# balbasty/torch-interpol

Hardware: AMD Instinct MI355X
Metric: Mvox/s grid_pull & grid_push, 256^3 fp32 cubic/dct2 (higher is better)
Workload: dtype f32

## Files before the change

torch-interpol_amd/csrc/push_owner.hip:

```cpp
#include "sorted_util.hpp"

namespace ip {
namespace owner {

using namespace sorted;

constexpr int BR = 16;
constexpr int OFF = 160;
constexpr int BOX = BR + 3;
constexpr int PZ = BOX;
constexpr int PLANE = BOX * PZ;
constexpr int BOXSLOTS = BOX * PLANE;
constexpr int NCELL = BR * BR * BR;
constexpr int CAPD = 128;
constexpr int CAPX = 512;
constexpr int NT = 512;
constexpr int NS = TS * TS * TS;
constexpr int NT1 = 512, VPT1 = NS / NT1;
constexpr int LB = 6, NBIN = LB * LB * LB;
constexpr int HDR_SHELL = 34;
constexpr int KMIX = 13;
template <int K> constexpr int KSV = K == KMIX ? 3 : K;
template <int K> __device__ __forceinline__ int kd(const KParams &p, int d) { return K == KMIX ? p.order[d] : K; }
#ifdef IP_OWNER_MIX_TU
// ... 870 lines not shown
#pragma unroll
        for (int d = 0; d < 3; ++d) wsum3 *= kd<K>(p, d) == 3 ? 1.6666667f : (kd<K>(p, d) == 2 ? 1.75f : 2.f);
        const bool dense = n >= 60000 || (float)(sm.dmax * foldmul) * wsum3 > 2147483648.f * 0.99f / magic_units_p<K>(p);
#else
        const float wsum = K == 3 ? 1.6666667f : (K == 2 ? 1.75f : 2.f);
        const bool dense = n >= 60000 || (float)(sm.dmax * foldmul) * (wsum * wsum * wsum) > magic_cbmax<K>();
#endif
        const bool one_batch = npieces <= NPIECE;
        for (int c = 0; c < nch; c += 2) {
            const bool two = c + 1 < nch;
            float *vc0 = vol + b * p.vol_sb + c * p.vol_sc;
            float *vc1 = two ? vc0 + p.vol_sc : vc0;
            const float *va = c == 0 ? nullptr : vals + (int64_t)(c - 1) * nrec;
            const float *vb = two ? vals + (int64_t)c * nrec : nullptr;
            if (c > 0) {
                float am0 = 0.f, am1 = 0.f;
                for (int e = tid; e < NCELL / 2; e += NT) sm.cells[e] = 0u;
                __syncthreads();
                for (int pb0 = 0; pb0 < npieces; pb0 += NPIECE) {
                    if (!one_batch) { __syncthreads(); build_pieces(pb0); }
                    for (int k = 0; k < VPT; ++k) {
                        const uint2 pc = sm.piece[wave + k * (NT / 64)];
                        if (lane >= (int)pc.y) continue;
                        const unsigned ri = pc.x + (unsigned)lane;
                        const int cell = (int)(meta[ri] & 4095u);
                        atomicAdd(&sm.cells[cell >> 1], 1u << (16 * (cell & 1)));
                        const float a0 = __builtin_fabsf(va[ri]), a1 = two ? __builtin_fabsf(vb[ri]) : 0.f;
                        am0 = (a0 > am0 || a0 != a0) ? a0 : am0;
                        am1 = (a1 > am1 || a1 != a1) ? a1 : am1;
                    }
                }
                const int w0 = wave_max(__float_as_int(am0)), w1 = wave_max(__float_as_int(am1));
                if (lane == 0) { if (w0) atomicMax(&sm.cmax[0], w0); if (w1) atomicMax(&sm.cmax[1], w1); }
                __syncthreads();
            }
            const int mb0 = sm.cmax[0], mb1 = sm.cmax[1];
            const bool fin = (mb0 & 0x7f800000) != 0x7f800000 && (mb1 & 0x7f800000) != 0x7f800000;
            const bool wide = dense && fin;
            const bool fixedpt = fin && !(p.dbg & 8);
            int ex0 = ((mb0 >> 23) & 0xff) - 127, ex1 = ((mb1 >> 23) & 0xff) - 127;
            ex0 = ex0 < -90 ? -90 : ex0; ex1 = ex1 < -90 ? -90 : ex1;
            const float a0 = fmaxf(__int_as_float(mb0), 1e-27f), a1 = fmaxf(__int_as_float(mb1), 1e-27f);
            const f2 scale = { mb0 ? IP_MU / a0 : 0.f, mb1 ? IP_MU / a1 : 0.f };
            const float inv0 = a0 * (1.f / IP_MU), inv1 = a1 * (1.f / IP_MU);
            const f2 scalew = { mb0 ? __int_as_float((127 + 30 - ex0) << 23) : 0.f, mb1 ? __int_as_float((127 + 30 - ex1) << 23) : 0.f };
            const float invw0 = __int_as_float((127 - 30 + ex0) << 23), invw1 = __int_as_float((127 - 30 + ex1) << 23);
            const unsigned boxaddr = (unsigned)(size_t)(__attribute__((address_space(3))) void *)(sm.box);
            for (int sub = 0; sub < (wide && two ? 2 : 1); ++sub) {
            for (int pb0 = 0; pb0 < npieces; pb0 += NPIECE) {
                const int tid = opaque((int)threadIdx.x);
                const int wave = tid >> 6, lane = tid & 63;
                if (pb0 > 0 || c > 0 || sub > 0) {
                    __syncthreads();
                    if (tid < NCLS) sm.qcnt[tid] = 0;
                    if (!one_batch) build_pieces(pb0); else __syncthreads();
#pragma unroll
                    for (int k = 0; k < VPT; ++k) {
                        const uint2 pc = sm.piece[wave + k * (NT / 64)];
                        qr[k] = -1;
                        if (lane < (int)pc.y) {
                            const unsigned mk = meta[pc.x + (unsigned)lane];
                            const int x0 = (mk >> 8) & 15, y0 = (mk >> 4) & 15, z0 = mk & 15;
                            const int q = (x0 * PLANE + y0 * PZ + z0) & (NCLS - 1);
                            qr[k] = q | (atomicAdd(&sm.qcnt[q], 1) << 4);
                        }
                    }
                    __syncthreads();
                } else if (!one_batch) {
                    __syncthreads();
                    build_pieces(0);
                }
                if (tid < 32) {
                    const bool cls = tid < NCLS;
                    const int cq = cls ? sm.qcnt[tid] : 0;
                    int tot, nsur, nhol;
                    half_excl_scan(cq, tot);
                    const int cap = (((tot + NCLS - 1) / NCLS) + NHW - 1) / NHW * NHW;
                    const int sur = cls && cq > cap ? cq - cap : 0, hol = cls && cq < cap ? cap - cq : 0;
                    const int so = half_excl_scan(sur, nsur), ho = half_excl_scan(hol, nhol);
                    if (cls) { sm.qsur[tid] = so; sm.qhol[tid] = ho; }
                    if (tid == 31) { sm.qsur[NCLS] = nsur; sm.qhol[NCLS] = nhol; sm.qcap = cap; }
                    const int fill = nsur - ho < 0 ? 0 : (nsur - ho > hol ? hol : nsur - ho);
                    if (cls) sm.qeff[tid] = (cq < cap ? cq : cap) + fill;
                }
                __syncthreads();
                const int qcap = sm.qcap;
#pragma unroll
                for (int k = 0; k < VPT; ++k) {
                    if (qr[k] < 0) continue;
                    const int qq = qr[k] & (NCLS - 1), r = qr[k] >> 4;
                    int slot = qq * qcap + r;
                    if (r >= qcap) {
                        const int o = sm.qsur[qq] + r - qcap;
                        int c2 = 0;
#pragma unroll
                        for (int st = NCLS / 2; st > 0; st >>= 1) if (sm.qhol[c2 + st] <= o) c2 += st;
                        slot = c2 * qcap + sm.qcnt[c2] + (o - sm.qhol[c2]);
                    }
                    sm.queue[slot] = (unsigned short)(((wave + k * (NT / 64)) << 6) | lane);
                }
                __syncthreads();
                const int q = tid & (NCLS - 1), hw = tid >> 4;
                const int ebeg = q * qcap + hw, eend = q * qcap + sm.qeff[q];
                const int nit = qcap / NHW;
                auto fetch = [&](int e, float4 &rc, float &s0, float &s1) {
                    const unsigned qe = sm.queue[e];
                    const unsigned ri = sm.piece[qe >> 6].x + (qe & 63u);
                    rc = rec[ri]; s0 = va ? va[ri] : rc.w; s1 = vb ? vb[ri] : 0.f;
                };
                float4 rc = make_float4(0.f, 0.f, 0.f, 0.f); float s0 = 0.f, s1 = 0.f;
                if (ebeg < eend) fetch(ebeg, rc, s0, s1);
#pragma unroll 1
                for (int it = 0; it < nit; ++it) {
                    const int e = ebeg + it * NHW;
                    const float4 cur = rc; const float cs0 = s0, cs1 = s1;
                    if (e + NHW < eend) fetch(e + NHW, rc, s0, s1);
                    if (e >= eend) continue;
                    int x0, y0, z0; float tx, ty, tz;
                    IP_RECORD_CELL(cur, b0, x0, y0, z0, tx, ty, tz);
                    if (fixedpt) {
#ifdef IP_ABLATE
                        if (p.dbg & 2) continue;
#endif
                        unsigned addr = boxaddr + 8u * (unsigned)(x0 * PLANE + y0 * PZ + z0);
                        f2 w[4];
#ifdef IP_OWNER_MIX_TU
                        if constexpr (K == KMIX) mixed_weights_yz(p.order[1], p.order[2], f2{ ty, tz }, w);
                        else
#endif
                        weights_yz<K>(f2{ ty, tz }, w);
                        if (wide) {
                            const f2 ss = sub ? f2{ cs1 * scalew.y, 0.f } : f2{ cs0 * scalew.x, 0.f };
                            scatter_plane<K, 0, true>(addr, ss, IP_WX(0), w, p.dbg);
                            scatter_plane<K, 1, true>(addr, ss, IP_WX(1), w, p.dbg);
                            if (IP_KS >= 2) scatter_plane<K, 2, true>(addr, ss, IP_WX(2), w, p.dbg);
                            if (IP_KS == 3) scatter_plane<K, 3, true>(addr, ss, IP_WX(3), w, p.dbg);
                        } else {
                            const f2 ss = f2{ cs0, cs1 } * scale;
                            scatter_plane<K, 0, false>(addr, ss, IP_WX(0), w, p.dbg);
                            scatter_plane<K, 1, false>(addr, ss, IP_WX(1), w, p.dbg);
                            if (IP_KS >= 2) scatter_plane<K, 2, false>(addr, ss, IP_WX(2), w, p.dbg);
                            if (IP_KS == 3) scatter_plane<K, 3, false>(addr, ss, IP_WX(3), w, p.dbg);
                        }
                    } else {
                        tiled::scatter_one_thread(L, vc0, cs0, b0[0] + x0, b0[1] + y0, b0[2] + z0, tx, ty, tz);
                        if (two) tiled::scatter_one_thread(L, vc1, cs1, b0[0] + x0, b0[1] + y0, b0[2] + z0, tx, ty, tz);
                    }
                }
            }
            asm volatile("s_waitcnt lgkmcnt(0)" ::: "memory");
            __syncthreads();
            prof_mark(11);
            const bool magic = fixedpt && !wide;
            if (magic) stencil_counts<K>(sm, tid);
            prof_mark(13);
            if (edge && fixedpt) {
#pragma unroll
                for (int d = 0; d < 3; ++d) {
                    const int nlo = b0[d] < 0 ? -b0[d] : 0, nhi = b0[d] + BOX > L.n[d] ? b0[d] + BOX - L.n[d] : 0;
                    if (nlo + nhi == 0) continue;
                    for (int i = tid; i < (nlo + nhi) * (BOX * BOX); i += NT) {
                        const int o = i / (BOX * BOX), rest = i - o * (BOX * BOX), r1 = rest / BOX, r2 = rest - r1 * BOX;
                        const int rd = o < nlo ? o : BOX - nhi + (o - nlo);
                        const int idx = b0[d] + rd;
                        int j;
                        if (L.bound[d] == B_REPLICATE) j = idx < 0 ? 0 : L.n[d] - 1;
                        else if (L.bound[d] == B_DCT1) j = idx < 0 ? -idx : 2 * L.n[d] - 2 - idx;
                        else j = idx < 0 ? -1 - idx : 2 * L.n[d] - 1 - idx;
                        const int rt = j - b0[d];
                        const int es = d == 0 ? rd * PLANE + r1 * PZ + r2 : d == 1 ? r1 * PLANE + rd * PZ + r2 : r1 * PLANE + r2 * PZ + rd;
                        const int et = d == 0 ? rt * PLANE + r1 * PZ + r2 : d == 1 ? r1 * PLANE + rt * PZ + r2 : r1 * PLANE + r2 * PZ + rt;
                        const unsigned long long v = sm.box[es];
                        if (v) { sm.box[es] = 0ull; atomicAdd(&sm.box[et], v); }
                        if (magic) {
                            const int ns = d == 0 ? (rd * BOX + r1) * NZ + r2 : d == 1 ? (r1 * BOX + rd) * NZ + r2 : (r1 * BOX + r2) * NZ + rd;
                            const int nt = d == 0 ? (rt * BOX + r1) * NZ + r2 : d == 1 ? (r1 * BOX + rt) * NZ + r2 : (r1 * BOX + r2) * NZ + rt;
                            unsigned short *nn = reinterpret_cast<unsigned short *>(sm.nreg);
                            const unsigned c2 = nn[ns];
                            if (c2) { nn[ns] = 0; atomicAdd(&sm.nreg[nt >> 1], c2 << (16 * (nt & 1))); }
                        }
                    }
                    __syncthreads();
                }
            }
            if (fixedpt && !atomic && !wide && !(p.dbg & 1)) {
                constexpr int UF2 = 7;
#pragma unroll 1
                for (int e0 = tid; e0 < BOXSLOTS; e0 += UF2 * NT) {
                    int off[UF2]; float t0[UF2], t1[UF2];
                    unsigned nz = 0, nst[UF2];
#pragma unroll
                    for (int u = 0; u < UF2; ++u) {
                        const int e = e0 + u * NT;
                        off[u] = 0;
                        if (e < BOXSLOTS) {
                            const int xr = e / PLANE, rem = e - xr * PLANE, yr = rem / PZ, zr = rem - yr * PZ;
                            off[u] = (b0[0] + xr) * L.ss[0] + (b0[1] + yr) * L.ss[1] + (b0[2] + zr) * L.ss[2];
                            nst[u] = stencils_at(sm, xr, yr, zr);
                            if (nst[u] != 0u) nz |= 1u << u;
                        }
                    }
#pragma unroll
                    for (int u = 0; u < UF2; ++u) {
                        t0[u] = ((nz >> u) & 1) ? vc0[off[u]] : 0.f;
                        t1[u] = (((nz >> u) & 1) && two) ? vc1[off[u]] : 0.f;
                    }
#pragma unroll
                    for (int u = 0; u < UF2; ++u) {
                        if (!((nz >> u) & 1)) continue;
                        const int e = e0 + u * NT;
                        const unsigned long long a = sm.box[e];
                        sm.box[e] = 0ull;
                        int lo_, hi_;
                        magic_decode(a, nst[u], lo_, hi_);
                        vc0[off[u]] = t0[u] + (float)lo_ * inv0;
                        if (two) vc1[off[u]] = t1[u] + (float)hi_ * inv1;
                    }
                }
            } else if (fixedpt && !(p.dbg & 1)) {
                constexpr int UF = 4;
                const int fl0 = atomic ? sm.rlo[0] : 0, fl1 = atomic ? sm.rlo[1] : 0, fl2 = atomic ? sm.rlo[2] : 0;
                const int fe1 = atomic ? sm.rhi[1] + IP_KS - fl1 + 1 : BOX, fe2 = atomic ? sm.rhi[2] + IP_KS - fl2 + 1 : BOX;
                const int nflush = atomic ? (sm.rhi[0] + IP_KS - fl0 + 1) * fe1 * fe2 : BOXSLOTS;
                const float r2 = 1.f / (float)fe2, r1 = 1.f / (float)fe1;
                for (int e0 = tid; e0 < nflush; e0 += UF * NT) {
                    long long a[UF]; int off[UF]; float sg[UF]; unsigned nst[UF];
#pragma unroll
                    for (int u = 0; u < UF; ++u) {
                        int e = e0 + u * NT;
                        a[u] = 0; off[u] = 0; sg[u] = 1.f; nst[u] = 0u;
                        if (e < nflush) {
                            int xr, yr, zr;
                            if (atomic) {
                                const int t = (int)(((float)e + 0.5f) * r2);
                                zr = e - t * fe2 + fl2;
                                xr = (int)(((float)t + 0.5f) * r1);
                                yr = t - xr * fe1 + fl1; xr += fl0;
                                e = xr * PLANE + yr * PZ + zr;
                            } else {
                                xr = e / PLANE; const int rem = e - xr * PLANE; yr = rem / PZ; zr = rem - yr * PZ;
                            }
                            a[u] = (long long)sm.box[e];
                            sm.box[e] = 0ull;
                            if (!wide) nst[u] = stencils_at(sm, xr, yr, zr);
                            if (atomic) {
                                off[u] = sm.taboff[0][xr] + sm.taboff[1][yr] + sm.taboff[2][zr];
                                sg[u] = sm.tabsgn[0][xr] * sm.tabsgn[1][yr] * sm.tabsgn[2][zr];
                            } else {
                                off[u] = (b0[0] + xr) * L.ss[0] + (b0[1] + yr) * L.ss[1] + (b0[2] + zr) * L.ss[2];
                            }
                        }
                    }
                    if (wide) {
                        float *vcs = sub ? vc1 : vc0;
                        const float invs = sub ? invw1 : invw0;
#pragma unroll
                        for (int u = 0; u < UF; ++u) {
                            if (a[u] == 0) continue;
                            const float val = (float)((double)a[u] * (double)(invs * sg[u]));
                            if (atomic) __hip_atomic_fetch_add(vcs + off[u], val, __ATOMIC_RELAXED, __HIP_MEMORY_SCOPE_AGENT);
                            else vcs[off[u]] += val;
                        }
                    } else if (atomic) {
#pragma unroll
                        for (int u = 0; u < UF; ++u) {
                            if (nst[u] == 0u) continue;
                            int lo_, hi_;
                            magic_decode((unsigned long long)a[u], nst[u], lo_, hi_);
                            if (lo_ != 0) __hip_atomic_fetch_add(vc0 + off[u], (float)lo_ * (inv0 * sg[u]), __ATOMIC_RELAXED, __HIP_MEMORY_SCOPE_AGENT);
                            if (hi_ != 0 && two) __hip_atomic_fetch_add(vc1 + off[u], (float)hi_ * (inv1 * sg[u]), __ATOMIC_RELAXED, __HIP_MEMORY_SCOPE_AGENT);
                        }
                    } else {
                        float t0[UF], t1[UF];
#pragma unroll
                        for (int u = 0; u < UF; ++u) {
                            t0[u] = nst[u] != 0u ? vc0[off[u]] : 0.f;
                            t1[u] = (nst[u] != 0u && two) ? vc1[off[u]] : 0.f;
                        }
#pragma unroll
                        for (int u = 0; u < UF; ++u) {
                            if (nst[u] == 0u) continue;
                            int lo_, hi_;
                            magic_decode((unsigned long long)a[u], nst[u], lo_, hi_);
                            vc0[off[u]] = t0[u] + (float)lo_ * inv0;
                            if (two) vc1[off[u]] = t1[u] + (float)hi_ * inv1;
                        }
                    }
                }
            }
            __syncthreads();
            }
            prof_mark(12);
            if (tid == 0) { sm.cmax[0] = 0; sm.cmax[1] = 0; }
        }
    }
    }
}

static __global__ void own_zero(int *__restrict__ p, int n)
{
    const int i = blockIdx.x * 1024 + threadIdx.x;
    if (i < n) p[i] = 0;
}


constexpr int GPZ = 20;
constexpr int GPLANE = BOX * GPZ;
struct GatSmem {
    int   taboff[3][BOX + 1];
    float tabsgn[3][BOX + 1];
    unsigned start[CAPD];
    int   pref[CAPD + 2];
    int   brick, pad;
    float2 box[BOX * GPLANE];
};
#define IP_RD(o, off) "ds_read_b64 %" #o ", %16 offset:" #off "\n\t"
__device__ __forceinline__ void gather_reads(unsigned addr, f2 (&v)[16])
{
    static_assert(GPZ * 8 == 160, "the immediate offsets are (row * GPZ + k) * 8");
    asm volatile(IP_RD(0, 0) IP_RD(1, 8) IP_RD(2, 16) IP_RD(3, 24)
                 IP_RD(4, 160) IP_RD(5, 168) IP_RD(6, 176) IP_RD(7, 184)
                 IP_RD(8, 320) IP_RD(9, 328) IP_RD(10, 336) IP_RD(11, 344)
                 IP_RD(12, 480) IP_RD(13, 488) IP_RD(14, 496) IP_RD(15, 504)
                 "s_waitcnt lgkmcnt(0)"
                 : "=&v"(v[0]), "=&v"(v[1]), "=&v"(v[2]), "=&v"(v[3]), "=&v"(v[4]), "=&v"(v[5]), "=&v"(v[6]), "=&v"(v[7]),
                   "=&v"(v[8]), "=&v"(v[9]), "=&v"(v[10]), "=&v"(v[11]), "=&v"(v[12]), "=&v"(v[13]), "=&v"(v[14]), "=&v"(v[15])
                 : "v"(addr) : "memory");
}
#undef IP_RD

template <int K, int GRAD = 0>
__global__ __launch_bounds__(NT, 4) void own_gather(KParams p, BrickGrid bg, const int *__restrict__ ndesc, const uint2 *__restrict__ desc,
                                                    const float4 *__restrict__ rec, const int *__restrict__ list, int *__restrict__ draw,
                                                    const float *__restrict__ img, float *__restrict__ out, const int *__restrict__ gate,
                                                    const float *__restrict__ gout)
{
    if (gate && *gate != 1) return;
    extern __shared__ __attribute__((aligned(16))) unsigned char smem_raw[];
    GatSmem &sm = *reinterpret_cast<GatSmem *>(smem_raw);
    const int nlist = list[0];
    for (;;) {
// ... 238 lines not shown
        if (!((valid >> v) & 1)) continue;
#pragma unroll
        for (int d = 0; d < 3; ++d) {
            const int i = fl[v][d] == fl[v][d] ? __float2int_rz(fl[v][d]) : 0;
            mn[d] = i < mn[d] ? i : mn[d]; mx[d] = i > mx[d] ? i : mx[d];
            if ((corner >> v) & 1) { atomicMin(&clo[d], i); atomicMax(&chi[d], i); }
        }
    }
#pragma unroll
    for (int d = 0; d < 3; ++d) {
        const int a = wave_min(mn[d]), e = wave_max(mx[d]);
        if ((tid & 63) == 0) { atomicMin(&lo[d], a); atomicMax(&hi[d], e); }
    }
    __syncthreads();
    const int cap[3] = { 33, 33, 32 };
    int l[3], h[3], boxvol = 1, cornervol = 1;
#pragma unroll
    for (int d = 0; d < 3; ++d) {
        int a = lo[d], sz = hi[d] + K - a + 1;
        if (sz > cap[d]) { a += (sz - cap[d]) / 2; sz = cap[d]; }
        l[d] = a; h[d] = a + sz - K - 1;
        boxvol *= sz > 0 ? sz : 0;
        const int cs = chi[d] + K - clo[d] + 1;
        cornervol *= cs > 0 ? (cs < cap[d] ? cs : cap[d]) : 0;
    }
    int slow = 0, nv = 0;
#pragma unroll
    for (int v = 0; v < VPT1; ++v) {
        if (!((valid >> v) & 1)) continue;
        ++nv;
        bool in = true;
#pragma unroll
        for (int d = 0; d < 3; ++d) {
            const int i = fl[v][d] == fl[v][d] ? __float2int_rz(fl[v][d]) : 0x7fffffff;
            in = in && i >= l[d] && i <= h[d];
        }
        if (!in) ++slow;
    }
    slow = wave_sum(slow); far = wave_sum(far); nv = wave_sum(nv);
    if ((tid & 63) == 0) { atomicAdd(&cnt[0], slow); atomicAdd(&cnt[1], far); atomicAdd(&cnt[2], nv); }
    __syncthreads();
    if (tid == 0) {
        atomicAdd(&hdr->nslow, cnt[0]); atomicAdd(&hdr->nfar, cnt[1]); atomicAdd(&hdr->nvalid, cnt[2]);
        if (cnt[2] == NS) { atomicAdd(&hdr->nbox, boxvol); atomicAdd(&hdr->nfull, 1); atomicAdd(&hdr->ncorner, cornervol); }
        __threadfence();
        if (atomicAdd(&hdr->done, 1) == (int)gridDim.x - 1) {
            const int ns = atomicAdd(&hdr->nslow, 0), nf = atomicAdd(&hdr->nfar, 0), nn = atomicAdd(&hdr->nvalid, 0);
            const int nb = atomicAdd(&hdr->nbox, 0), nt = atomicAdd(&hdr->nfull, 0), nc = atomicAdd(&hdr->ncorner, 0);
            const bool rough = nch > 1 && (int64_t)nb > (int64_t)BOXVOL * nt && (int64_t)nb * 10 > (int64_t)nc * 16;
            const bool dense = (int64_t)nc <= (int64_t)DENSEVOL * nt;
            if (nch == -2) hdr->gate = ((int64_t)ns * 1000 > (int64_t)nn * PULLOUT && (int64_t)nf * 64 <= nn) ? 1 : 0;
            else if (nch < 0) hdr->gate = (((int64_t)ns * 250 > nn || dense) && (int64_t)nf * 64 <= nn) ? 1 : 0;
            else hdr->gate = (((int64_t)ns * 250 > nn || rough) && (int64_t)nf * 64 <= nn) ? 1 : 0;
        }
    }
}

struct Workspace {
    int *flags;
    ProbeHdr *hdr; int *ndesc; int *bmax; uint2 *desc; float4 *rec; float *vals; unsigned short *meta;
    int64_t nrec; int nbricks;
};
static int64_t align256(int64_t x) { return (x + 255) & ~(int64_t)255; }

static int64_t layout(const KParams &k, int B, int ntiles, int nch, void *base, Workspace *w, int64_t nflags = 0, bool shared = false)
{
    const BrickGrid bg = brick_grid(k);
    const int64_t nbricks = (int64_t)bg.per_item * (shared ? 1 : B);
    const int64_t nrec = (int64_t)ntiles * NS * B;
    int64_t o = 0;
    unsigned char *p = (unsigned char *)base;
    const int64_t o_hdr = o; o += 256;
    const int64_t o_nd = o; o += nbricks * 4;
    const int64_t o_bm = o; o += nbricks * 8;
    const int64_t o_fl = o; o += nflags * 4; o = align256(o);
    const int64_t o_desc = o; o += align256(nbricks * (shared ? CAPX : CAPD) * 8);
    const int64_t o_rec = o; o += align256(nrec * 16);
    const int64_t o_val = o; o += align256(nrec * 4 * (nch > 1 ? nch - 1 : 0));
    const int64_t o_meta = o; o += align256(nrec * 2);
    if (w) {
        w->hdr = (ProbeHdr *)(p + o_hdr); w->ndesc = (int *)(p + o_nd); w->desc = (uint2 *)(p + o_desc);
        w->rec = (float4 *)(p + o_rec); w->vals = (float *)(p + o_val); w->meta = (unsigned short *)(p + o_meta);
        w->bmax = (int *)(p + o_bm); w->flags = (int *)(p + o_fl);
        w->nrec = nrec; w->nbricks = (int)nbricks;
    }
    return o;
}

static int tile_count(const interpol_problem *p)
{
    int64_t n = 1;
    for (int d = 0; d < 3; ++d) n *= (p->grid_shape[d] + TS - 1) / TS;
    return n > 0x7fffffff ? 0 : (int)n;
}

int mix_launch_bin(int dtype, int idx, const KParams &k, const BrickGrid &bg, const Workspace &w, const void *val, const void *grid, void *vol,
                   const int *gate, const void *aux, const int *all, int gx, int gy, int gz, int ntiles, int B, hipStream_t st);
int mix_launch_acc(const KParams &k, const BrickGrid &bg, const Workspace &w, void *vol, int nch, int color, int Bw, const int *gate,
                   unsigned nblocks, hipStream_t st);
int mix_launch_gather(int grad, const KParams &k, const BrickGrid &bg, const Workspace &w, const void *vol, void *val, const int *gate,
                      const void *gout, unsigned nblocks, hipStream_t st);

#ifdef IP_OWNER_MIX_TU
int mix_launch_bin(int dtype, int idx, const KParams &k, const BrickGrid &bg, const Workspace &w, const void *val, const void *grid, void *vol,
                   const int *gate, const void *aux, const int *all, int gx, int gy, int gz, int ntiles, int B, hipStream_t st)
{
    const int nty = (gy + TS - 1) / TS, ntz = (gz + TS - 1) / TS;
    const dim3 tgrid((unsigned)(ntiles * B));
#define IP_MIX_BIN(T, IDX)                                                                                              \
    {                                                                                                                   \
        const int attr = big_lds<own_bin<T, KMIX, 0, IDX>>(sizeof(BinSmem));                                            \
        if (attr) return attr;                                                                                          \
        hipLaunchKernelGGL((own_bin<T, KMIX, 0, IDX>), tgrid, dim3(NT1), sizeof(BinSmem), st, k, bg, (const T *)val, (const float *)grid, \
                           (float *)vol, w.ndesc, w.desc, w.rec, w.vals, w.meta, w.bmax, w.nrec, gx, gy, gz, nty, ntz, ntiles, gate, (const T *)aux, all); \
    }
    if (idx == 0) { if (dtype == INTERPOL_F32) IP_MIX_BIN(float, 0) else if (dtype == INTERPOL_BF16) IP_MIX_BIN(bf16_t, 0) else if (dtype == INTERPOL_F16) IP_MIX_BIN(f16_t, 0) else return INTERPOL_E_DTYPE; }
    else if (idx == 1) IP_MIX_BIN(float, 1) else if (idx == 2) IP_MIX_BIN(float, 2) else IP_MIX_BIN(float, 3)
#undef IP_MIX_BIN
    const hipError_t e = hipGetLastError();
    return e == hipSuccess ? 0 : (int)e;
}
int mix_launch_acc(const KParams &k, const BrickGrid &bg, const Workspace &w, void *vol, int nch, int color, int Bw, const int *gate,
                   unsigned nblocks, hipStream_t st)
{
    const int attr = big_lds<own_accumulate<KMIX>>(sizeof(AccSmem));
    if (attr) return attr;
    hipLaunchKernelGGL((own_accumulate<KMIX>), dim3(nblocks), dim3(NT), sizeof(AccSmem), st, k, bg, (const int *)w.ndesc,
                       (const uint2 *)w.desc, (const float4 *)w.rec, (const float *)w.vals, (const unsigned short *)w.meta,
                       (const int *)w.bmax, w.nrec, (float *)vol, nch, color, Bw, gate, (int *)w.hdr + 16 + color);
    const hipError_t e = hipGetLastError();
    return e == hipSuccess ? 0 : (int)e;
}
int mix_launch_gather(int grad, const KParams &k, const BrickGrid &bg, const Workspace &w, const void *vol, void *val, const int *gate,
                      const void *gout, unsigned nblocks, hipStream_t st)
{
#define IP_MIX_GAT(GR)                                                                                                  \
    {                                                                                                                   \
        const int attr = big_lds<own_gather<KMIX, GR>>(sizeof(GatSmem));                                                \
        if (attr) return attr;                                                                                          \
        hipLaunchKernelGGL((own_gather<KMIX, GR>), dim3(nblocks), dim3(NT), sizeof(GatSmem), st, k, bg, (const int *)w.ndesc, (const uint2 *)w.desc, \
                           (const float4 *)w.rec, (const int *)w.bmax, (int *)w.hdr + 40, (const float *)vol, (float *)val, gate, (const float *)gout); \
    }
    if (grad == 1) IP_MIX_GAT(1) else if (grad == 2) IP_MIX_GAT(2) else IP_MIX_GAT(0)
#undef IP_MIX_GAT
    const hipError_t e = hipGetLastError();
    return e == hipSuccess ? 0 : (int)e;
}
#endif

}

#ifndef IP_OWNER_MIX_TU

static bool shared_target(const interpol_problem *p) { return p->vol_stride[0] == 0 && p->batch > 1; }
static bool mixed_orders(const KParams &k) { return k.order[0] != k.order[1] || k.order[0] != k.order[2]; }
static bool owner_eligible(const interpol_problem *p, const KParams &k, bool scatter = false)
{
    const bool shared = scatter && shared_target(p);
    if (p->dim != 3 || p->batch > 4096) return false;
    if (!(p->flags & (INTERPOL_FLAG_BINNED_SCATTER | INTERPOL_FLAG_AUTO_SCATTER))) return false;
    if (k.order[0] != k.order[1] || k.order[0] != k.order[2]) {
        for (int d = 0; d < 3; ++d) if (k.order[d] < 1 || k.order[d] > 3) return false;
        if (k.sep != 0) return false;
    } else if (k.order[0] < (scatter ? 1 : 2) || k.order[0] > 3) return false;
    int64_t n = 1, nv = 1, nb = shared ? 1 : p->batch;
    for (int d = 0; d < 3; ++d) {
        n *= p->grid_shape[d]; nv *= p->vol_shape[d];
        nb *= owner::NLO + owner::NHI + (p->vol_shape[d] + 15 + owner::BR - 1) / owner::BR;
        if (p->grid_shape[d] > 0x7fffffff / 4) return false;
    }
    const int64_t nt = owner::tile_count(p);
    if (n < 4096 || nt == 0 || nt * owner::NS * p->batch > 0x7fffffffll || nb > 0x7fffffffll / (shared ? owner::CAPX : owner::CAPD)) return false;
    if ((uint64_t)n * 12ull > 0xffffffffull) return false;
    return (shared ? 8 * n * p->batch : 4 * n) >= nv;
}

int linear_pull_probe(const interpol_problem *p, const KParams &k, const void *grid, void *workspace, hipStream_t st, const int **gate_out, int thr16);
constexpr int NEAREST_THR16 = 24;
static bool nearest_scatter(const KParams &k) { return k.dim == 3 && k.mode == MODE_ISO0 && k.order[0] == 0 && k.order[1] == 0 && k.order[2] == 0; }
static KParams nearest_as_trilinear(const KParams &k)
{
    KParams q = k;
    if (nearest_scatter(k)) { q.order[0] = 1; q.order[1] = 1; q.order[2] = 1; }
    return q;
}

int64_t owner_workspace_bytes(const interpol_problem *p, const KParams &k_in, bool count_only)
{
    const KParams k = nearest_as_trilinear(k_in);
    if (!owner_eligible(p, k, true)) return 0;
    const int nch = count_only ? 1 : k.C + (k.cc ? 1 : 0);
    return owner::layout(k, (int)p->batch, owner::tile_count(p), nch, nullptr, nullptr, 0, shared_target(p));
}

namespace owner {
template <typename T, int IDX = 0>
static int launch_bin(const interpol_problem *p, const KParams &k, const BrickGrid &bg, const Workspace &w, const void *val, const void *grid,
                      void *vol, const int *gate, hipStream_t st, const void *aux = nullptr, const int *all = nullptr)
{
    const int gx = (int)p->grid_shape[0], gy = (int)p->grid_shape[1], gz = (int)p->grid_shape[2];
    const int nty = (gy + TS - 1) / TS, ntz = (gz + TS - 1) / TS;
    const int ntiles = tile_count(p);
    const dim3 tgrid((unsigned)(ntiles * (int)p->batch));
    if (k.order[0] != k.order[1] || k.order[0] != k.order[2])
        return mix_launch_bin(std::is_same<T, float>::value ? INTERPOL_F32 : (std::is_same<T, bf16_t>::value ? INTERPOL_BF16 : INTERPOL_F16), IDX, k, bg, w,
                              val, grid, vol, gate, aux, all, gx, gy, gz, ntiles, (int)p->batch, st);
#define IP_OWN_BIN(KK, GM)                                                                                              \
    {                                                                                                                   \
        const int attr = big_lds<own_bin<T, KK, GM, IDX>>(sizeof(BinSmem));                                               \
        if (attr) return attr;                                                                                          \
        hipLaunchKernelGGL((own_bin<T, KK, GM, IDX>), tgrid, dim3(NT1), sizeof(BinSmem), st, k, bg, (const T *)val, (const float *)grid, \
                           (float *)vol, w.ndesc, w.desc, w.rec, w.vals, w.meta, w.bmax, w.nrec, gx, gy, gz, nty, ntz, ntiles, gate, (const T *)aux, all); \
    }
#define IP_OWN_BY_GM(KK)                                                                                                \
    { if (k.sep == 0) IP_OWN_BIN(KK, 0) else if (k.sep == 1) IP_OWN_BIN(KK, 1) else if (k.sep == 2) IP_OWN_BIN(KK, 2) else IP_OWN_BIN(KK, 3) }
    if (k.order[0] == 3) IP_OWN_BY_GM(3) else if (k.order[0] == 2) IP_OWN_BY_GM(2) else IP_OWN_BY_GM(1)
#undef IP_OWN_BY_GM
#undef IP_OWN_BIN
    return 0;
}
}

int try_owner_push(const interpol_problem *p, const KParams &k_in, const void *val, const void *grid, void *vol,
                   void *workspace, int64_t workspace_bytes, hipStream_t st, const int **gate_out)
{
    using namespace owner;
    const bool nearest = nearest_scatter(k_in);
    const KParams k = nearest_as_trilinear(k_in);
    if (!workspace || !owner_eligible(p, k, true)) return 0;
    const bool count_only = val == nullptr;
    const int nch = count_only ? 1 : k.C + (k.cc ? 1 : 0);
    Workspace w;
    if (((uintptr_t)workspace & 255u) != 0) return 0;
    const bool shared = shared_target(p);
    if (layout(k, (int)p->batch, tile_count(p), nch, workspace, &w, 0, shared) > workspace_bytes) return 0;
    BrickGrid bg = brick_grid(k);
    if (shared) { bg.item = 0; bg.capd = CAPX; }
    const bool gated = !(p->flags & INTERPOL_FLAG_BINNED_SCATTER);
    if (nearest && gated && k.sep != 0 && k.sep != 2) return 0;
    hipLaunchKernelGGL(own_zero, dim3((unsigned)((64 + 3ll * w.nbricks + 1023) / 1024)), dim3(1024), 0, st, (int *)w.hdr, 64 + 3 * w.nbricks);
    hipError_t e = hipGetLastError();
    if (e != hipSuccess) return (int)e;
    const int *gate = nullptr;
    const int B = (int)p->batch;
    if (gated && nearest) {
        const int rp = linear_pull_probe(p, k, grid, w.hdr, st, &gate, NEAREST_THR16);
        if (rp) return rp;
    } else if (gated) {
        const int gx = (int)p->grid_shape[0], gy = (int)p->grid_shape[1], gz = (int)p->grid_shape[2];
        const int nty = (gy + TS - 1) / TS, ntz = (gz + TS - 1) / TS, ntiles = tile_count(p);
        const long long total = (long long)ntiles * B;
        const dim3 pgrid((unsigned)(total < NPROBE ? total : NPROBE));
#define IP_OWN_PROBE(KK, GM) hipLaunchKernelGGL((own_probe<KK, GM>), pgrid, dim3(NT1), 0, st, k, bg, (const float *)grid, w.hdr, gx, gy, gz, nty, ntz, ntiles, B, nch);
#define IP_OWN_PROBE_GM(KK) { if (k.sep == 0) IP_OWN_PROBE(KK, 0) else if (k.sep == 1) IP_OWN_PROBE(KK, 1) else if (k.sep == 2) IP_OWN_PROBE(KK, 2) else IP_OWN_PROBE(KK, 3) }
        if (k.order[0] == 3 || mixed_orders(k)) IP_OWN_PROBE_GM(3) else if (k.order[0] == 2) IP_OWN_PROBE_GM(2) else IP_OWN_PROBE_GM(1)
#undef IP_OWN_PROBE_GM
#undef IP_OWN_PROBE
        gate = &w.hdr->gate;
    }
    int rc;
    switch (count_only ? INTERPOL_F32 : p->dtype) {
    case INTERPOL_F32: rc = launch_bin<float>(p, k, bg, w, val, grid, vol, gate, st); break;
    case INTERPOL_BF16: rc = launch_bin<bf16_t>(p, k, bg, w, val, grid, vol, gate, st); break;
    case INTERPOL_F16: rc = launch_bin<f16_t>(p, k, bg, w, val, grid, vol, gate, st); break;
    default: return 0;
    }
    if (rc) return rc;
    const long long want = 2ll * cu_count();
    const int Bw = shared ? 1 : B;
    for (int color = 0; color < 9; ++color) {
        long long nwork = Bw;
        for (int d = 0; d < 3; ++d) nwork *= color_count(color, d, bg);
        if (nwork <= 0) continue;
        const dim3 agrid((unsigned)(nwork < want ? nwork : want));
#define IP_OWN_ACC(KK)                                                                                                  \
        {                                                                                                               \
            const int attr = big_lds<own_accumulate<KK>>(sizeof(AccSmem));                                              \
            if (attr) return attr;                                                                                      \
            hipLaunchKernelGGL((own_accumulate<KK>), agrid, dim3(NT), sizeof(AccSmem), st, k, bg, (const int *)w.ndesc,  \
                               (const uint2 *)w.desc, (const float4 *)w.rec, (const float *)w.vals, (const unsigned short *)w.meta,  \
                               (const int *)w.bmax, w.nrec, (float *)vol, nch, color, Bw, gate, \
                               (int *)w.hdr + 16 + color);                                                              \
        }
        if (mixed_orders(k)) { const int rm = mix_launch_acc(k, bg, w, vol, nch, color, Bw, gate, agrid.x, st); if (rm) return rm; }
        else if (k.order[0] == 3) IP_OWN_ACC(3) else if (k.order[0] == 2) IP_OWN_ACC(2)
        else if (nearest) {
            const int attr = big_lds<own_accumulate<1, true>>(sizeof(AccSmem));
            if (attr) return attr;
            hipLaunchKernelGGL((own_accumulate<1, true>), agrid, dim3(NT), sizeof(AccSmem), st, k, bg, (const int *)w.ndesc,
                               (const uint2 *)w.desc, (const float4 *)w.rec, (const float *)w.vals, (const unsigned short *)w.meta,
                               (const int *)w.bmax, w.nrec, (float *)vol, nch, color, Bw, gate, (int *)w.hdr + 16 + color);
        }
        else IP_OWN_ACC(1)
#undef IP_OWN_ACC
    }
    e = hipGetLastError();
    if (e != hipSuccess) return (int)e;
    if (gate_out) *gate_out = gate;
    return gated ? 2 : 1;
}

static bool owner_pull_eligible(const interpol_problem *p, const KParams &k)
{
    if (p->dtype != INTERPOL_F32 || p->grid_dtype != INTERPOL_F32) return false;
    if (p->val_stride[0] < 0) return false;
    return owner_eligible(p, k);
}
int64_t owner_pull_workspace_bytes(const interpol_problem *p, const KParams &k)
{
    if (!owner_pull_eligible(p, k)) return 0;
    const int nt = owner::tile_count(p);
    return owner::layout(k, (int)p->batch, nt, 1, nullptr, nullptr, (int64_t)nt * p->batch);
}
int owner_pull_prepare(const interpol_problem *p, const KParams &k, void *workspace, int64_t workspace_bytes, hipStream_t st, int **flags_out, int *nzero_out)
{
    using namespace owner;
    if (!workspace || !owner_pull_eligible(p, k)) return 0;
    if (((uintptr_t)workspace & 255u) != 0) return 0;
    const int nt = tile_count(p);
    const int64_t nflags = (int64_t)nt * p->batch;
    Workspace w;
    if (layout(k, (int)p->batch, nt, 1, workspace, &w, nflags) > workspace_bytes) return 0;
    const int64_t nz = 64 + 3ll * w.nbricks;
    if (nz + nflags > 0x7fffffffll || (int *)w.hdr + nz != w.flags) return 0;
    if (p->flags & INTERPOL_FLAG_BINNED_SCATTER) {
        hipLaunchKernelGGL(own_zero, dim3((unsigned)((nz + 1023) / 1024)), dim3(1024), 0, st, (int *)w.hdr, (int)nz);
        const hipError_t e = hipGetLastError();
        if (e != hipSuccess) return (int)e;
    }
    *flags_out = w.flags;
    *nzero_out = (int)nz;
    return 1;
}
int owner_grad_probe(const interpol_problem *p, const KParams &k, const void *grid, void *workspace, int64_t workspace_bytes, hipStream_t st, int mode)
{
    using namespace owner;
    const int ntiles = tile_count(p);
    Workspace w;
    if (layout(k, (int)p->batch, ntiles, 1, workspace, &w, (int64_t)ntiles * p->batch) > workspace_bytes) return INTERPOL_E_SCRATCH;
    const BrickGrid bg = brick_grid(k);
    const int64_t nz = 64 + 3ll * w.nbricks;
    hipLaunchKernelGGL(own_zero, dim3((unsigned)((nz + 1023) / 1024)), dim3(1024), 0, st, (int *)w.hdr, (int)nz);
    const int B = (int)p->batch;
    const int gx = (int)p->grid_shape[0], gy = (int)p->grid_shape[1], gz = (int)p->grid_shape[2];
    const int nty = (gy + TS - 1) / TS, ntz = (gz + TS - 1) / TS;
    const long long total = (long long)ntiles * B;
    const dim3 pgrid((unsigned)(total < NPROBE ? total : NPROBE));
#define IP_OWN_PROBE(KK, GM) hipLaunchKernelGGL((own_probe<KK, GM>), pgrid, dim3(NT1), 0, st, k, bg, (const float *)grid, w.hdr, gx, gy, gz, nty, ntz, ntiles, B, mode);
#define IP_OWN_PROBE_GM(KK) { if (k.sep == 0) IP_OWN_PROBE(KK, 0) else if (k.sep == 1) IP_OWN_PROBE(KK, 1) else if (k.sep == 2) IP_OWN_PROBE(KK, 2) else IP_OWN_PROBE(KK, 3) }
    if (k.order[0] == 3 || mixed_orders(k)) IP_OWN_PROBE_GM(3) else IP_OWN_PROBE_GM(2)
#undef IP_OWN_PROBE_GM
#undef IP_OWN_PROBE
    const hipError_t e = hipGetLastError();
    return e == hipSuccess ? 0 : (int)e;
}
namespace owner {
template <int GM>
__global__ __launch_bounds__(256) void lin_probe(KParams p, const float *__restrict__ grid, int *__restrict__ hdr, int gx, int gy, int gz, int nty, int ntz,
                                                 int ntiles, long long total, int stride, int thr16)
{
    __shared__ int acc[2];
    const int tid = threadIdx.x;
    if (tid < 2) acc[tid] = 0;
    __syncthreads();
    const long long work = (long long)blockIdx.x * stride;
    const long long wk = work < total ? work : total - 1;
    const int64_t b = wk / ntiles;
    const TileGeom g = tile_geom((int)(wk % ntiles), gx, gy, gz, nty, ntz);
    float s = 0.f; int n = 0;
    for (int id = tid; id < TS * TS * TS; id += 512) {
        int ox, oy, oz;
        sample_pos(g, id, ox, oy, oz);
        if (ox >= gx || oy >= gy || oz + 2 >= gz || (id & 15) + 2 >= TS) continue;
        float q0[3], q1[3], q2[3];
        load_xyz<GM>(p, grid, b, g, ox, oy, oz, q0);
        load_xyz<GM>(p, grid, b, g, ox, oy, oz + 1, q1);
        load_xyz<GM>(p, grid, b, g, ox, oy, oz + 2, q2);
        for (int d = 0; d < 3; ++d) s += __builtin_fabsf(q0[d] - 2.f * q1[d] + q2[d]);
        ++n;
    }
    s = s < 1e4f ? s : 1e4f;
    if (n) { atomicAdd(&acc[0], (int)(s * 16.f)); atomicAdd(&acc[1], n); }
    __syncthreads();
    if (tid == 0) {
        const unsigned long long a0 = (unsigned long long)(acc[0] < (1 << 20) ? acc[0] : (1 << 20)), a1 = (unsigned long long)acc[1];
        const unsigned long long add = work < total ? (a0 << 34) | (a1 << 12) | 1ull : 1ull;
        const unsigned long long tot = __hip_atomic_fetch_add(reinterpret_cast<unsigned long long *>(hdr + 2), add, __ATOMIC_RELAXED, __HIP_MEMORY_SCOPE_AGENT) + add;
        if ((tot & 0xfffull) == (unsigned long long)gridDim.x) {
            const unsigned long long sum16 = tot >> 34, cnt = (tot >> 12) & 0x3fffffull;
            __hip_atomic_store(&hdr[0], (cnt > 0 && sum16 > cnt * (unsigned long long)thr16) ? 1 : 0, __ATOMIC_RELAXED, __HIP_MEMORY_SCOPE_AGENT);
        }
    }
}

}

int linear_pull_probe(const interpol_problem *p, const KParams &k, const void *grid, void *workspace, hipStream_t st, const int **gate_out, int thr16)
{
    using namespace owner;
    int *hdr = (int *)workspace;
    hipLaunchKernelGGL(own_zero, dim3(1), dim3(64), 0, st, hdr, 8);
    const int gx = (int)p->grid_shape[0], gy = (int)p->grid_shape[1], gz = (int)p->grid_shape[2];
    const int ntx = (gx + TS - 1) / TS, nty = (gy + TS - 1) / TS, ntz = (gz + TS - 1) / TS, ntiles = ntx * nty * ntz;
    const long long total = (long long)ntiles * p->batch;
    int stride = (int)((total + 511) / 512);
    stride = stride < 1 ? 1 : (stride | 1);
    const unsigned nb = (unsigned)((total + stride - 1) / stride);
    if (k.sep == 0) hipLaunchKernelGGL((lin_probe<0>), dim3(nb), dim3(256), 0, st, k, (const float *)grid, hdr, gx, gy, gz, nty, ntz, ntiles, total, stride, thr16);
    else hipLaunchKernelGGL((lin_probe<2>), dim3(nb), dim3(256), 0, st, k, (const float *)grid, hdr, gx, gy, gz, nty, ntz, ntiles, total, stride, thr16);
    *gate_out = hdr;
    const hipError_t e = hipGetLastError();
    return e == hipSuccess ? 0 : (int)e;
}

int owner_pull_finish(const interpol_problem *p, const KParams &k, const void *vol, const void *grid, void *val,
                      void *workspace, int64_t workspace_bytes, bool all, hipStream_t st, bool grad, const void *gout, bool probed, bool spatial)
{
    using namespace owner;
    const int nt = tile_count(p);
    Workspace w;
    if (layout(k, (int)p->batch, nt, 1, workspace, &w, (int64_t)nt * p->batch) > workspace_bytes) return INTERPOL_E_SCRATCH;
    const BrickGrid bg = brick_grid(k);
    KParams kk = k;
    kk.gate = nullptr;
    int rc = grad ? launch_bin<float, 2>(p, kk, bg, w, vol, grid, val, all ? nullptr : w.flags, st, gout, probed ? &w.hdr->gate : nullptr)
           : spatial ? launch_bin<float, 3>(p, kk, bg, w, vol, grid, val, nullptr, st, nullptr, probed ? &w.hdr->gate : nullptr)
                  : launch_bin<float, 1>(p, kk, bg, w, vol, grid, val, all ? nullptr : w.flags, st, nullptr, probed ? &w.hdr->gate : nullptr);
    if (rc) return rc;
    const long long want = 2ll * cu_count();
    const dim3 ggrid((unsigned)(w.nbricks < want ? w.nbricks : want));
#define IP_OWN_GAT(KK, GR)                                                                                              \
    {                                                                                                                   \
        const int attr = big_lds<own_gather<KK, GR>>(sizeof(GatSmem));                                                  \
        if (attr) return attr;                                                                                          \
        hipLaunchKernelGGL((own_gather<KK, GR>), ggrid, dim3(NT), sizeof(GatSmem), st, kk, bg, (const int *)w.ndesc, (const uint2 *)w.desc, \
                           (const float4 *)w.rec, (const int *)w.bmax, (int *)w.hdr + 40, (const float *)vol, (float *)val,            \
                           (spatial && probed) ? (const int *)&w.hdr->gate : (const int *)nullptr, (const float *)gout);  \
    }
    if (mixed_orders(k)) {
        const int rm = mix_launch_gather(grad ? 1 : (spatial ? 2 : 0), kk, bg, w, vol, val, (spatial && probed) ? (const int *)&w.hdr->gate : (const int *)nullptr, gout, ggrid.x, st);
        if (rm) return rm;
    }
// ... 28 lines not shown
```

Before: 31380.

## Add float4 row-vectorized flush path for owner accumulate behind dbg flag

Adds an alternative flush of the LDS fixed-point box to global memory in own_accumulate. Each row's interior is handled as aligned float4 quads, and the three leftover z slots per row are handled as scalar edge elements. The goal is fewer global load/store instructions and better coalescing. The path only runs when dbg bit 8192 is set and the host confirms alignment via rows_flushable. By default dbg likely lacks that bit, so the existing UF2 loop still runs; that loop now only takes opaque(tid).

```diff
diff --git a/torch-interpol_amd/csrc/push_owner.hip b/torch-interpol_amd/csrc/push_owner.hip
--- a/torch-interpol_amd/csrc/push_owner.hip
+++ b/torch-interpol_amd/csrc/push_owner.hip
@@ -1046,7 +1046,7 @@
             __syncthreads();
             prof_mark(11);
             const bool magic = fixedpt && !wide;
-            if (magic) stencil_counts<K>(sm, tid);
+            if (magic) stencil_counts<K>(sm, opaque(tid));
             prof_mark(13);
             if (edge && fixedpt) {
 #pragma unroll
@@ -1077,10 +1077,76 @@
                     __syncthreads();
                 }
             }
-            if (fixedpt && !atomic && !wide && !(p.dbg & 1)) {
+            if (fixedpt && !atomic && !wide && (p.dbg & (1 | 8192)) == 8192) {
+                constexpr int NROW = BOX * BOX, NQUAD = 4 * NROW, NEND = 3 * NROW, QR = 2;
+                const int ft = opaque(tid), hd = (-opaque(b0[2])) & 3;
+#pragma unroll 1
+                for (int i0 = ft; i0 < NQUAD; i0 += QR * NT) {
+                    int off[QR], eoff[QR]; unsigned n01[QR], n23[QR], ns[QR]; float4 t0[QR], t1[QR]; float s0[QR], s1[QR];
+#pragma unroll
+                    for (int u = 0; u < QR; ++u) {
+                        const int i = i0 + u * NT;
+                        {
+                            const int iq = i < NQUAD ? i : NQUAD - 1;
+                            const int row = iq >> 2, zr = hd + 4 * (iq & 3), xr = row / BOX, yr = row - xr * BOX;
+                            off[u] = (b0[0] + xr) * L.ss[0] + (b0[1] + yr) * L.ss[1] + b0[2] + zr;
+                            const unsigned *nr = sm.nreg + row * (NZ / 2) + (zr >> 1);
+                            const unsigned d0 = nr[0], d1 = nr[1], d2 = nr[2];
+                            n01[u] = i < NQUAD ? __builtin_amdgcn_alignbit(d1, d0, 16u * (hd & 1)) : 0u;
+                            n23[u] = i < NQUAD ? __builtin_amdgcn_alignbit(d2, d1, 16u * (hd & 1)) : 0u;
+                        }
+                        {
+                            const int ie = i < NEND ? i : NEND - 1;
+                            const int s = (ie >= NROW ? 1 : 0) + (ie >= 2 * NROW ? 1 : 0), row = ie - s * NROW, zr = s < hd ? s : s + 16;
+                            const int xr = row / BOX, yr = row - xr * BOX;
+                            eoff[u] = (b0[0] + xr) * L.ss[0] + (b0[1] + yr) * L.ss[1] + b0[2] + zr;
+                            const unsigned n = i < NEND ? stencils_at(sm, xr, yr, zr) : 0u;
+                            ns[u] = n != 0u ? n | (unsigned)(row * PZ + zr) << 16 : 0u;
+                        }
+                        if ((n01[u] | n23[u]) == 0u) off[u] = 0;
+                        if (ns[u] == 0u) eoff[u] = 0;
+                    }
+#pragma unroll
+                    for (int u = 0; u < QR; ++u) {
+                        t0[u] = *reinterpret_cast<const float4 *>(vc0 + off[u]);
+                        if (two) t1[u] = *reinterpret_cast<const float4 *>(vc1 + off[u]);
+                        s0[u] = vc0[eoff[u]];
+                        if (two) s1[u] = vc1[eoff[u]];
+                    }
+#pragma unroll
+                    for (int u = 0; u < QR; ++u) {
+                        if ((n01[u] | n23[u]) != 0u) {
+                            const int i = i0 + u * NT;
+                            unsigned long long *s = sm.box + (i >> 2) * PZ + hd + 4 * (i & 3);
+                            const unsigned nn[4] = { n01[u] & 0xffffu, n01[u] >> 16, n23[u] & 0xffffu, n23[u] >> 16 };
+                            float r0[4] = { t0[u].x, t0[u].y, t0[u].z, t0[u].w }, r1[4] = { t1[u].x, t1[u].y, t1[u].z, t1[u].w };
+#pragma unroll
+                            for (int j = 0; j < 4; ++j) {
+                                const unsigned long long a = s[j];
+                                s[j] = 0ull;
+                                int lo_, hi_;
+                                magic_decode(a, nn[j], lo_, hi_);
+                                r0[j] = nn[j] != 0u ? r0[j] + (float)lo_ * inv0 : r0[j];
+                                r1[j] = nn[j] != 0u ? r1[j] + (float)hi_ * inv1 : r1[j];
+                            }
+                            *reinterpret_cast<float4 *>(vc0 + off[u]) = make_float4(r0[0], r0[1], r0[2], r0[3]);
+                            if (two) *reinterpret_cast<float4 *>(vc1 + off[u]) = make_float4(r1[0], r1[1], r1[2], r1[3]);
+                        }
+                        if (ns[u] != 0u) {
+                            const int e = (int)(ns[u] >> 16);
+                            const unsigned long long a = sm.box[e];
+                            sm.box[e] = 0ull;
+                            int lo_, hi_;
+                            magic_decode(a, ns[u] & 0xffffu, lo_, hi_);
+                            vc0[eoff[u]] = s0[u] + (float)lo_ * inv0;
+                            if (two) vc1[eoff[u]] = s1[u] + (float)hi_ * inv1;
+                        }
+                    }
+                }
+            } else if (fixedpt && !atomic && !wide && !(p.dbg & 1)) {
                 constexpr int UF2 = 7;
 #pragma unroll 1
-                for (int e0 = tid; e0 < BOXSLOTS; e0 += UF2 * NT) {
+                for (int e0 = opaque(tid); e0 < BOXSLOTS; e0 += UF2 * NT) {
                     int off[UF2]; float t0[UF2], t1[UF2];
                     unsigned nz = 0, nst[UF2];
 #pragma unroll
@@ -1625,6 +1691,11 @@
 
 #ifndef IP_OWNER_MIX_TU
 
+static bool rows_flushable(const KParams &k, const void *vol)
+{
+    return k.vol_ss[2] == 4 && k.vol_ss[0] % 16 == 0 && k.vol_ss[1] % 16 == 0 && k.vol_n[2] % 4 == 0
+        && k.vol_sb % 4 == 0 && k.vol_sc % 4 == 0 && (uintptr_t)vol % 16 == 0;
+}
 static bool shared_target(const interpol_problem *p) { return p->vol_stride[0] == 0 && p->batch > 1; }
 static bool mixed_orders(const KParams &k) { return k.order[0] != k.order[1] || k.order[0] != k.order[2]; }
 static bool owner_eligible(const interpol_problem *p, const KParams &k, bool scatter = false)
@@ -1741,6 +1812,8 @@
     if (rc) return rc;
     const long long want = 2ll * cu_count();
     const int Bw = shared ? 1 : B;
+    KParams ka = k;
+    if (!rows_flushable(k, vol)) ka.dbg &= ~8192;
     for (int color = 0; color < 9; ++color) {
         long long nwork = Bw;
         for (int d = 0; d < 3; ++d) nwork *= color_count(color, d, bg);
@@ -1750,17 +1823,17 @@
         {                                                                                                               \
             const int attr = big_lds<own_accumulate<KK>>(sizeof(AccSmem));                                              \
             if (attr) return attr;                                                                                      \
-            hipLaunchKernelGGL((own_accumulate<KK>), agrid, dim3(NT), sizeof(AccSmem), st, k, bg, (const int *)w.ndesc,  \
+            hipLaunchKernelGGL((own_accumulate<KK>), agrid, dim3(NT), sizeof(AccSmem), st, ka, bg, (const int *)w.ndesc,  \
                                (const uint2 *)w.desc, (const float4 *)w.rec, (const float *)w.vals, (const unsigned short *)w.meta,  \
                                (const int *)w.bmax, w.nrec, (float *)vol, nch, color, Bw, gate, \
                                (int *)w.hdr + 16 + color);                                                              \
         }
-        if (mixed_orders(k)) { const int rm = mix_launch_acc(k, bg, w, vol, nch, color, Bw, gate, agrid.x, st); if (rm) return rm; }
+        if (mixed_orders(k)) { const int rm = mix_launch_acc(ka, bg, w, vol, nch, color, Bw, gate, agrid.x, st); if (rm) return rm; }
         else if (k.order[0] == 3) IP_OWN_ACC(3) else if (k.order[0] == 2) IP_OWN_ACC(2)
         else if (nearest) {
             const int attr = big_lds<own_accumulate<1, true>>(sizeof(AccSmem));
             if (attr) return attr;
-            hipLaunchKernelGGL((own_accumulate<1, true>), agrid, dim3(NT), sizeof(AccSmem), st, k, bg, (const int *)w.ndesc,
+            hipLaunchKernelGGL((own_accumulate<1, true>), agrid, dim3(NT), sizeof(AccSmem), st, ka, bg, (const int *)w.ndesc,
                                (const uint2 *)w.desc, (const float4 *)w.rec, (const float *)w.vals, (const unsigned short *)w.meta,
                                (const int *)w.bmax, w.nrec, (float *)vol, nch, color, Bw, gate, (int *)w.hdr + 16 + color);
         }
```

After: 31710 (median of 6 runs). 1.0% higher.
